# fjdf/slaMEM

Measured on AMD Instinct MI355X. Metric: MEMs/sec (and queries/sec) on 100 Mbp ref x 10 M 150 bp queries, l=20, higher is better.
Workload: dtype u32; 1 GPU; synthetic 100000000 bp reference (splitmix64 seed 42) x 10000000 reads/GPU of 150 bp, 2% substitutions, 50% reverse-complemented, -b -l 20; ref_len=100000000, reads_total=10000000, read_len=150, min_len=20, both_strands=True, parallelism=query shards x1, one GPU, no replication

## Files before the change

slamem_amd/csrc/mem_search.hip:

```cpp
#include "common.h"
#include "prims.h"

#include <atomic>
#include <type_traits>
#include <new>
#include <stdlib.h>
#include <string.h>

namespace slamem {

struct Blk {
    uint4 a;
    uint4 b;
    uint4 c;
    uint4 d;
};

__device__ __forceinline__ uint64_t u64_of(uint32_t lo, uint32_t hi) { return ((uint64_t)hi << 32) | lo; }

__device__ __forceinline__ Blk load_blk(const FMBlock* __restrict__ fm, uint32_t bi) {
    const uint4* p = reinterpret_cast<const uint4*>(fm + bi);
    Blk k;
    k.a = p[0]; k.b = p[1]; k.c = p[2]; k.d = p[3];
    return k;
// ... 102 lines not shown
struct SearchArgs {
    IndexView ix;
    const uint64_t* qwords;
    const uint64_t* offsets;
    uint32_t num_queries;
    uint32_t strands;
    uint32_t min_len;
    int32_t pad0;
    uint32_t pad1;
    uint32_t pad;
    uint64_t capacity;
    unsigned long long* total;
    RawKey* raw_key;
    slamem_mem* raw_mem;
    uint32_t* block_counts;
    struct RawRow* inline_rows;
    uint64_t inline_stride;
    const struct ItemDesc* items;
    uint64_t num_items;
    uint8_t* item_attempt;
    const uint8_t* item_alive;
    const uint32_t* work_ids;
    const uint32_t* work_count;
    unsigned long long* stats;
    uint64_t query_words;
    const uint64_t* pq;
    uint64_t* pq_out;
    uint32_t implicit_items;
    uint32_t* seed_left_ids;
    unsigned int* seed_left_count;
    unsigned int* seed_long_flag;
    unsigned int* seed_wide;
    uint32_t seed_step;
    const uint64_t* item_pk;
    unsigned int* work_cursor;
    int32_t direct_min_depth;
    uint32_t use_jump;
    uint32_t pad2;
    uint32_t skip_w;
    const uint64_t* pq2;
    uint64_t* pq2_out;
    uint8_t* item_flags;
    uint32_t skip_s1;
    uint32_t pad4;
    const struct SliceState* slice_state;
    const uint32_t* item_block;
    struct OutCtx {
        struct RawRow* inline_rows;
        uint64_t inline_stride;
        RawKey* raw_key;
        slamem_mem* raw_mem;
        unsigned long long* total;
        uint64_t capacity;
        uint32_t* block_counts;
        uint8_t* item_attempt;
    } prev;
    struct DeferCtx {
        struct JobRec* queue;
        unsigned int* njobs;
        uint32_t* pool;
        unsigned int* pool_next;
        uint32_t pool_cap;
        uint32_t queue_cap;
        uint32_t epoch;
        uint32_t* raw_seg;
        uint2* list;
        unsigned int* nlist;
        uint8_t* inline_valid;
    } defer;
    const struct CarryRec* carry_in;
    const unsigned int* carry_in_count;
    struct CarryRec* carry_out;
    unsigned int* carry_out_count;
};

struct RawRow { uint32_t row, pos, len; };
constexpr uint32_t kInlineMems = 4;
constexpr uint32_t kFetch = 64;

constexpr uint32_t kSliceLen = 4096;
static_assert(kSliceLen == kSearchSliceLen, "stream.hip tells the slice count of a batch from this length");
constexpr uint32_t kWarmUp = 1024;
constexpr uint32_t kMaxAttempt = 7;
struct __attribute__((aligned(16))) ItemDesc {
    uint64_t base;
    uint32_t len;
    uint32_t slice_rev;
};
__device__ __forceinline__ ItemDesc item_of(const SearchArgs& A, uint64_t it) {
    if (!A.implicit_items) return A.items[it];
    const uint64_t q = A.strands == 2u ? it >> 1 : it;
    const uint64_t o0 = A.offsets[q];
    return ItemDesc{o0, (uint32_t)(A.offsets[q + 1] - o0), A.strands == 2u ? (uint32_t)(it & 1ull) << 31 : 0u};
}
__device__ __forceinline__ uint64_t item_pk_of(const SearchArgs& A, uint64_t it, const ItemDesc& d) {
    if (!A.implicit_items) return A.item_pk[it];
    const uint64_t q = A.strands == 2u ? it >> 1 : it;
    const uint64_t rel = d.base - A.offsets[0];
    return 2ull + (uint64_t)A.strands * 2ull * ((rel >> 5) + q) + (uint64_t)(d.slice_rev >> 31) * 2ull * ((d.len + 31u) >> 5);
}

template <uint32_t kBytes>
struct QueryCursorT {
    const uint64_t* words;
    uint64_t base;
    uint32_t len;
    uint32_t rev;
    uint64_t cidx;
    uint64_t q0, q1, q2, q3;
    __device__ __forceinline__ void init(const uint64_t* q, uint64_t b, uint32_t l, uint32_t r) {
        words = q; base = b; len = l; rev = r; cidx = ~0ull;
// ... 2320 lines not shown
                    for (uint32_t wi = (af + s - 1u) / s, wl = (bf - k) / s; wi <= wl; wi++) {
                        const uint32_t x = st ? Lj - k - wi * s : wi * s;
                        uint64_t word = 0ull;
#pragma unroll
                        for (int w = 0; w < (int)NW; w++) word = (x >> 6) == (uint32_t)w ? uqs[w] : word;
                        if ((word >> (x & 63u)) & 1ull) done |= 1ull << wi;
                    }
                    if (done) atomicOr(&S.expl[jr], done);
                }
            }
            if (kStats) {
                const uint32_t nh = (uint32_t)__popcll(__ballot(has));
                n_cmp += nh;
                if (mark && lane == 0u) atomicAdd(A.stats + SC_SEED_ONCE, (unsigned long long)nh);
            }
            const unsigned long long mb = __ballot(is_mem);
            if (is_mem) {
                const uint32_t at = nmems + (uint32_t)__popcll(mb & below);
                if (at < SeedWave<NW, R>::kMems) { S.mem_key[at] = key; S.mem_ref[at] = ref; S.mem_sig[at] = sig | ((2u * jr + st) << 25); }
                else { atomicOr(&S.flags, 1u << jr); if (kStats) atomicAdd(A.stats + SC_SEED_WHY + 5u, 1ull); }
            }
            nmems += (uint32_t)__popcll(mb);
        }
        wave_sync();
    };

    for (uint32_t round = 0; round < (mstep > 1u ? 2u : 1u); round++) {
        njobs = 0;
        lookups(round);
        compares(round);
    }
    };
    if (wave_hasn) search(std::true_type{}); else search(std::false_type{});
    {
        if (nmems > SeedWave<NW, R>::kMems) nmems = SeedWave<NW, R>::kMems;

        const uint32_t g0 = (uint32_t)(r0 * strands);
        auto rank_of = [&](uint32_t mi, uint32_t key, uint32_t g, uint32_t& rank, uint32_t& cnt, bool& tie) {
            rank = 0; cnt = 0; tie = false;
            for (uint32_t t2 = 0; t2 < nmems; t2++) {
                const uint32_t kk = S.mem_key[t2], gg = S.mem_sig[t2] >> 25;
                const bool same = gg == g;
                cnt += same ? 1u : 0u;
                rank += (same && kk > key) ? 1u : 0u;
                tie = tie || (same && kk == key && t2 != mi);
            }
        };
        auto tie_rank = [&](uint32_t mi, uint32_t key, uint32_t myref, uint32_t g, uint32_t sig, uint32_t& rank) -> bool {
            const uint32_t a = key >> 16, b = a + (key & 0xFFFFu);
            bool child = false;
            for (uint32_t t2 = 0; t2 < nmems; t2++) {
                const uint32_t kk = S.mem_key[t2], a2 = kk >> 16, b2 = a2 + (kk & 0xFFFFu);
                child = child || ((S.mem_sig[t2] >> 25) == g && kk != key && a2 <= a && b2 > b);
            }
            const uint32_t jr = g >> 1, st = g & 1u;
            uint32_t qb = 0;
            if (child) qb = (uint32_t)((S.pl[jr][st][0][b >> 6] >> (b & 63u)) & 1ull) | ((uint32_t)((S.pl[jr][st][1][b >> 6] >> (b & 63u)) & 1ull) << 1);
            auto letter = [&](uint32_t sg, uint32_t t) { return ((sg >> t) & 1u) | (((sg >> (t + kSigLetters)) & 1u) << 1); };
            const bool rows = ix.prec != nullptr;
            const uint32_t my_side = child && letter(sig, 0u) > qb ? 1u : 0u;
            bool bad = (sig & kSigKnown) == 0u && (child || !rows);
            for (uint32_t t2 = 0; t2 < nmems; t2++) {
                const uint32_t so = S.mem_sig[t2];
                if (t2 == mi || (so >> 25) != g || S.mem_key[t2] != key) continue;
                const bool known = (so & sig & kSigKnown) != 0u;
                if (!known && (child || !rows)) { bad = true; continue; }
                const uint32_t o_side = child && letter(so, 0u) > qb ? 1u : 0u;
                bool before;
                if (o_side != my_side) before = o_side == 0u;
                else {
                    const uint32_t x = sig ^ so, diff = known ? (x | (x >> kSigLetters)) & kSigMask : 0u;
                    bool smaller;
                    if (diff != 0u) {
                        const uint32_t t = (uint32_t)__ffs((int)diff) - 1u;
                        smaller = letter(so, t) < letter(sig, t);
                    } else if (rows) smaller = ix.prec[S.mem_ref[t2]].row < ix.prec[myref].row;
                    else { bad = true; continue; }
                    before = my_side == 0u ? smaller : !smaller;
                }
                rank += before ? 1u : 0u;
            }
            return bad;
        };
        auto emit_mem = [&](uint32_t fl, uint32_t key, uint32_t ref, uint32_t gb, uint32_t rank, uint32_t cnt) {
            if ((fl >> (gb >> 1)) & 1u) return;
            const uint32_t g = g0 + (strands == 2u ? gb : gb >> 1);
            emit3_at(A, g, rank, 0u, ref, key >> 16, (key & 0xFFFFu) | 0x80000000u);
            if (rank == 0u) A.block_counts[g] = cnt;
            if (kStats) n_mem++;
        };
        if (nmems <= 64u) {
            const bool has = lane < nmems;
            const uint32_t key = has ? S.mem_key[lane] : 0u, ref = has ? S.mem_ref[lane] : 0u, g = has ? S.mem_sig[lane] >> 25 : 0xFFFFFFFFu;
            if (lane < 2u * R) S.smask[lane] = 0ull;
            wave_sync();
            if (has) atomicOr(&S.smask[g], 1ull << lane);
            wave_sync();
            const unsigned long long mine = has ? S.smask[g] : 0ull;
            uint32_t rank = 0;
            const uint32_t cnt = (uint32_t)__popcll(mine);
            bool tie = false;
            for (unsigned long long o = mine & ~(1ull << lane); __ballot(o != 0ull) != 0ull; o &= o - 1ull) {
                if (o == 0ull) continue;
                const uint32_t kk = S.mem_key[__ffsll(o) - 1];
                rank += kk > key ? 1u : 0u;
                tie = tie || kk == key;
            }
            if (has && tie && tie_rank(lane, key, ref, g, S.mem_sig[lane], rank)) {
                atomicOr(&S.flags, 1u << (g >> 1));
                if (kStats) atomicAdd(A.stats + SC_SEED_WHY + 6u, 1ull);
            }
            wave_sync();
            if (has) emit_mem(S.flags | wflags, key, ref, g, rank, cnt);
        } else {
            for (uint32_t pass = 0; pass < 2u; pass++) {
                const uint32_t fl = pass ? (S.flags | wflags) : 0u;
                for (uint32_t m0i = 0; m0i < nmems; m0i += 64u) {
                    const uint32_t mi = m0i + lane;
                    const bool has = mi < nmems;
                    const uint32_t key = has ? S.mem_key[mi] : 0u, ref = has ? S.mem_ref[mi] : 0u, g = has ? S.mem_sig[mi] >> 25 : 0xFFFFFFFFu;
                    uint32_t rank, cnt;
                    bool tie;
                    rank_of(mi, key, g, rank, cnt, tie);
                    const bool bad = has && tie && tie_rank(mi, key, ref, g, S.mem_sig[mi], rank);
                    if (!pass) { if (bad) atomicOr(&S.flags, 1u << (g >> 1)); }
                    else if (has) emit_mem(fl, key, ref, g, rank, cnt);
                }
                wave_sync();
            }
        }
    }
    wave_sync();
    const uint32_t fl = S.flags | wflags;
    {
        const bool isleft = lane < nr * strands && ((fl >> (strands == 2u ? lane >> 1 : lane)) & 1u) != 0u;
        if (lane < nr * strands) alive[r0 * strands + lane] = isleft ? 1 : 0;
        const unsigned long long lm = __ballot(isleft);
        if (lm != 0ull) {
            unsigned int at = 0;
            if (lane == 0u) at = atomicAdd(A.seed_left_count, (unsigned int)__popcll(lm));
            at = (unsigned int)__builtin_amdgcn_readfirstlane((int)at);
            if (isleft) A.seed_left_ids[at + (uint32_t)__popcll(lm & below)] = (uint32_t)(r0 * strands + lane);
        }
    }
    if (kStats) {
        stat_flush<kStats>(A.stats + SC_SEED_NMASKS, n_nm);
        stat_flush<kStats>(A.stats + SC_SEED_MEMS, n_mem);
        if (lane == 0u) {
            atomicAdd(A.stats + SC_SEED_WINDOWS, (unsigned long long)n_win);
            atomicAdd(A.stats + SC_SEED_COMPARES, (unsigned long long)n_cmp);
            atomicAdd(A.stats + SC_SEED_READS, (unsigned long long)nr);
            atomicAdd(A.stats + SC_SEED_QBYTES, (unsigned long long)(__builtin_amdgcn_readlane((int)(uint32_t)off, (int)nr) - __builtin_amdgcn_readlane((int)(uint32_t)off, 0)));
            atomicAdd(A.stats + SC_SEED_LEFT, (unsigned long long)(strands * (uint32_t)__popc(fl)));
            atomicAdd(A.stats + SC_SEED_WHY + 0u, (unsigned long long)__popc(wflags));
        }
    }
}

__global__ void __launch_bounds__(256) k_place_inline(const RawRow* __restrict__ inl, uint64_t stride, const uint32_t* __restrict__ counts,
                                                      const uint64_t* __restrict__ item_off, uint64_t nitems,
                                                      const uint32_t* __restrict__ sa, uint64_t capacity,
                                                      slamem_mem* __restrict__ out, const uint8_t* __restrict__ inline_valid) {
    uint64_t g = (uint64_t)blockIdx.x * blockDim.x + threadIdx.x;
    if (g >= nitems) return;
    uint32_t cnt = counts[g];
    uint64_t off = item_off[g];
    uint32_t iv = inline_valid ? inline_valid[g] : 0u;
    asm volatile("" : "+v"(cnt), "+v"(off), "+v"(iv));
    if (cnt > kInlineMems) cnt = kInlineMems;
    if (iv && cnt > iv - 1u) cnt = iv - 1u;
    if (cnt == 0u) return;
    static_assert(kInlineMems == 4, "k_place_inline is written for four inline slots");
    const RawRow* in = inl + g;
    const RawRow none = {0u, 0u, 0x80000000u};
    RawRow r0 = in[0], r1 = none, r2 = none, r3 = none;
    if (cnt > 1u) r1 = in[stride];
    if (cnt > 2u) r2 = in[2u * stride];
    if (cnt > 3u) r3 = in[3u * stride];
    asm volatile("" : "+v"(r0.row), "+v"(r0.pos), "+v"(r0.len), "+v"(r1.row), "+v"(r1.pos), "+v"(r1.len));
    asm volatile("" : "+v"(r2.row), "+v"(r2.pos), "+v"(r2.len), "+v"(r3.row), "+v"(r3.pos), "+v"(r3.len));
    uint32_t p0 = r0.row, p1 = r1.row, p2 = r2.row, p3 = r3.row;
    if (!(r0.len >> 31)) p0 = sa[r0.row];
    if (cnt > 1u && !(r1.len >> 31)) p1 = sa[r1.row];
    if (cnt > 2u && !(r2.len >> 31)) p2 = sa[r2.row];
    if (cnt > 3u && !(r3.len >> 31)) p3 = sa[r3.row];
    asm volatile("" : "+v"(p0), "+v"(p1), "+v"(p2), "+v"(p3));
    if (off < capacity) out[off] = slamem_mem{p0, r0.pos, r0.len & 0x7FFFFFFFu};
    if (cnt > 1u && off + 1u < capacity) out[off + 1u] = slamem_mem{p1, r1.pos, r1.len & 0x7FFFFFFFu};
    if (cnt > 2u && off + 2u < capacity) out[off + 2u] = slamem_mem{p2, r2.pos, r2.len & 0x7FFFFFFFu};
    if (cnt > 3u && off + 3u < capacity) out[off + 3u] = slamem_mem{p3, r3.pos, r3.len & 0x7FFFFFFFu};
}

__global__ void __launch_bounds__(256) k_group_totals(const uint32_t* __restrict__ counts, uint64_t nitems, uint64_t* __restrict__ totals) {
    const uint64_t g = (uint64_t)blockIdx.x * blockDim.x + threadIdx.x;
    uint64_t v = g < nitems ? (uint64_t)counts[g] : 0ull;
#pragma unroll
    for (int d = 32; d > 0; d >>= 1) v += u64_of(__shfl_down((uint32_t)v, d), __shfl_down((uint32_t)(v >> 32), d));
    if ((threadIdx.x & 63u) == 0u && (g >> 6) <= (nitems >> 6)) totals[g >> 6] = v;
}
__global__ void __launch_bounds__(256) k_place_grouped(const uint32_t* __restrict__ counts, uint64_t nitems, const uint64_t* __restrict__ group_prefix,
                                                       uint64_t* __restrict__ block_offsets, const RawRow* __restrict__ inl, uint64_t stride,
                                                       const uint32_t* __restrict__ sa, uint64_t capacity, slamem_mem* __restrict__ out,
                                                       const uint8_t* __restrict__ inline_valid) {
    const uint64_t g = (uint64_t)blockIdx.x * blockDim.x + threadIdx.x;
    const uint32_t lane = threadIdx.x & 63u;
    const bool item = g < nitems;
    const uint32_t full = item ? counts[g] : 0u;
    uint32_t iv = (item && inline_valid) ? inline_valid[g] : 0u;
    uint64_t gp = g <= nitems ? group_prefix[g >> 6] : 0ull;
    RawRow r0 = {0u, 0u, 0x80000000u};
    if (full != 0u) r0 = inl[g];
    asm volatile("" : "+v"(iv), "+v"(gp), "+v"(r0.row), "+v"(r0.pos), "+v"(r0.len));
    uint64_t incl = full;
#pragma unroll
    for (int d = 1; d < 64; d <<= 1) {
        const uint64_t o = u64_of(__shfl_up((uint32_t)incl, d), __shfl_up((uint32_t)(incl >> 32), d));
        if ((int)lane >= d) incl += o;
    }
    const uint64_t off = gp + (incl - full);
    if (g <= nitems) block_offsets[g] = off;
    uint32_t cnt = full > kInlineMems ? kInlineMems : full;
    if (iv && cnt > iv - 1u) cnt = iv - 1u;
    if (cnt == 0u) return;
    static_assert(kInlineMems == 4, "k_place_grouped is written for four inline slots");
    const RawRow none = {0u, 0u, 0x80000000u};
    RawRow r1 = none, r2 = none, r3 = none;
    if (cnt > 1u) r1 = inl[stride + g];
    if (cnt > 2u) r2 = inl[2u * stride + g];
    if (cnt > 3u) r3 = inl[3u * stride + g];
    asm volatile("" : "+v"(r1.row), "+v"(r1.pos), "+v"(r1.len), "+v"(r2.row), "+v"(r2.pos), "+v"(r2.len), "+v"(r3.row), "+v"(r3.pos), "+v"(r3.len));
    uint32_t p0 = r0.row, p1 = r1.row, p2 = r2.row, p3 = r3.row;
    if (!(r0.len >> 31)) p0 = sa[r0.row];
    if (cnt > 1u && !(r1.len >> 31)) p1 = sa[r1.row];
    if (cnt > 2u && !(r2.len >> 31)) p2 = sa[r2.row];
    if (cnt > 3u && !(r3.len >> 31)) p3 = sa[r3.row];
    asm volatile("" : "+v"(p0), "+v"(p1), "+v"(p2), "+v"(p3));
    if (off < capacity) out[off] = slamem_mem{p0, r0.pos, r0.len & 0x7FFFFFFFu};
    if (cnt > 1u && off + 1u < capacity) out[off + 1u] = slamem_mem{p1, r1.pos, r1.len & 0x7FFFFFFFu};
    if (cnt > 2u && off + 2u < capacity) out[off + 2u] = slamem_mem{p2, r2.pos, r2.len & 0x7FFFFFFFu};
    if (cnt > 3u && off + 3u < capacity) out[off + 3u] = slamem_mem{p3, r3.pos, r3.len & 0x7FFFFFFFu};
}

__global__ void __launch_bounds__(256) k_place_overflow(const RawKey* __restrict__ key, const slamem_mem* __restrict__ raw,
                                                        const unsigned long long* __restrict__ listed,
                                                        const uint64_t* __restrict__ item_off,
                                                        const uint8_t* __restrict__ item_attempt,
                                                        const uint32_t* __restrict__ sa, uint64_t capacity,
                                                        slamem_mem* __restrict__ out, const uint32_t* __restrict__ raw_seg,
                                                        const uint32_t* __restrict__ pool) {
    uint64_t count = *listed;
    if (count > capacity) count = capacity;
    const uint64_t stride = (uint64_t)gridDim.x * blockDim.x;
    for (uint64_t i = (uint64_t)blockIdx.x * blockDim.x + threadIdx.x; i < count; i += stride) {
        RawKey kk = key[i];
        if (kk.block == 0xFFFFFFFFu) continue;
        if ((kk.k >> 28) != item_attempt[kk.block]) continue;
        slamem_mem m = raw[i];
        uint64_t pos = item_off[kk.block] + (kk.k & 0x0FFFFFFFu);
        if (raw_seg) {
            const uint32_t sg = raw_seg[i];
            if (sg != 0xFFFFFFFFu) pos += pool[sg];
        }
        if (pos >= capacity) continue;
        if (m.length >> 31) m.length &= 0x7FFFFFFFu;
        else m.ref_pos = sa[m.ref_pos];
        out[pos] = m;
    }
}

__global__ void __launch_bounds__(256) k_item_counts(const uint64_t* __restrict__ offsets, uint32_t nq, uint32_t slice_len,
                                                     uint32_t* __restrict__ cnt, uint32_t* __restrict__ wps,
                                                     unsigned int* __restrict__ most) {
    uint64_t q = (uint64_t)blockIdx.x * blockDim.x + threadIdx.x;
    uint32_t c = 0, w = 0;
    if (q < nq) {
// ... 57 lines not shown
    uint32_t t = top[i], b = bot[i];
    if (t > b || b > ix.n) { depth_out[i] = -2; return; }
    depth_out[i] = parent(ix, t, b);
    top[i] = t;
    bot[i] = b;
}

__global__ void __launch_bounds__(256) k_locate_batch(IndexView ix, const uint32_t* __restrict__ rows, uint32_t* out,
                                                      uint64_t count) {
    uint64_t i = (uint64_t)blockIdx.x * blockDim.x + threadIdx.x;
    if (i >= count) return;
    uint32_t r = rows[i];
    out[i] = r <= ix.n ? ix.sa[r] : 0xFFFFFFFFu;
}

__global__ void __launch_bounds__(256) k_bwtchar_batch(IndexView ix, const uint32_t* __restrict__ rows, char* out,
                                                       uint64_t count) {
    uint64_t i = (uint64_t)blockIdx.x * blockDim.x + threadIdx.x;
    if (i >= count) return;
    uint32_t r = rows[i];
    const char L[] = {'$', 'N', 'A', 'C', 'G', 'T'};
    out[i] = r <= ix.n ? L[bwt_code(ix, r)] : '?';
}

namespace {
inline unsigned grid_for(uint64_t items, unsigned block = 256) { return (unsigned)((items + block - 1) / block); }
inline uint64_t align_up(uint64_t x, uint64_t a) { return (x + a - 1) / a * a; }

constexpr uint64_t kK8Waves = 4096;
constexpr uint64_t kCarryLanes = kK8Waves * 64;

struct WorkspaceLayout {
    uint64_t off_total, off_cnt, off_first, off_scan32, off_items, off_counts, off_attempt, off_alive, off_workids, off_select, select_bytes, off_itemoff, off_gsum, off_gpre, off_rawkey,
        off_rawmem, off_inline, off_scan, scan_bytes, off_wps, off_wscan, off_itempk, off_pq, pq_bytes, off_pq2, off_itemflags, off_mamstate, off_mamrun, off_itemblock, off_slicestate, off_carry, off_defscal, off_jobq, off_pool, off_rawseg, off_deflist, pool_cap, max_bounds, max_items, bytes;
};

WorkspaceLayout layout_workspace(uint64_t num_queries, uint64_t strands, uint64_t query_bytes, uint64_t capacity) {
    WorkspaceLayout w;
    w.max_items = strands * (num_queries + query_bytes / kSliceLen + 1);
    uint64_t off = 0;
    w.off_total = off;    off = align_up(off + 64 + SC_COUNT * 8, 256);
    w.off_cnt = off;      off = align_up(off + (num_queries + 2) * 4, 256);
    w.off_first = off;    off = align_up(off + (num_queries + 2) * 4, 256);
    w.off_scan32 = off;   off = align_up(off + scan_u32_tmp_words(num_queries + 1) * 4, 256);
    w.off_items = off;    off = align_up(off + w.max_items * sizeof(ItemDesc), 256);
    w.off_counts = off;   off = align_up(off + (w.max_items + 1) * 4, 256);
    w.off_attempt = off;  off = align_up(off + w.max_items, 256);
    w.off_alive = off;    off = align_up(off + w.max_items, 256);
    w.off_workids = off;  off = align_up(off + w.max_items * 4, 256);
    {
        size_t need2 = 0;
        (void)select_indices_u32(nullptr, need2, nullptr, nullptr, nullptr, w.max_items, 0);
        w.select_bytes = need2;
        w.off_select = off;
        off = align_up(off + need2, 256);
    }
    w.off_itemoff = off;  off = align_up(off + (w.max_items + 1) * 8, 256);
    w.off_gsum = off;     off = align_up(off + ((w.max_items >> 6) + 2) * 8, 256);
    w.off_gpre = off;     off = align_up(off + ((w.max_items >> 6) + 2) * 8, 256);
    w.off_rawkey = off;   off = align_up(off + capacity * sizeof(RawKey), 256);
    w.off_rawmem = off;   off = align_up(off + capacity * sizeof(slamem_mem), 256);
    w.off_inline = off;   off = align_up(off + w.max_items * kInlineMems * sizeof(RawRow), 256);
    size_t need = 0;
    (void)scan_sum_exclusive_u32_u64(nullptr, need, nullptr, nullptr, w.max_items, 0);
    w.scan_bytes = need;
    w.off_scan = off;     off = align_up(off + need, 256);
    w.off_wps = off;      off = align_up(off + (num_queries + 2) * 4, 256);
    w.off_wscan = off;    off = align_up(off + (num_queries + 2) * 8, 256);
    w.off_itempk = off;   off = align_up(off + w.max_items * 8, 256);
    w.pq_bytes = 8 * (4 + strands * (query_bytes / 16 + 2 * num_queries + 2));
    w.off_pq = off;       off = align_up(off + w.pq_bytes, 256);
    w.off_pq2 = off;      off = align_up(off + w.pq_bytes / 2 + 64, 256);
    w.off_itemflags = off; off = align_up(off + w.max_items, 256);
    w.max_bounds = strands * (query_bytes / kSliceLen + 1);
    w.off_mamstate = off; off = align_up(off + 2 * w.max_bounds * sizeof(MamState), 256);
    w.off_mamrun = off;   off = align_up(off + w.max_bounds * 4, 256);
    w.off_itemblock = off; off = align_up(off + w.max_items * 4, 256);
    w.off_slicestate = off; off = align_up(off + w.max_bounds * sizeof(SliceState), 256);
    w.off_carry = off;    off = align_up(off + kCarryLanes * sizeof(CarryRec), 256);
    w.pool_cap = strands * (query_bytes + 6 * num_queries) + 64;
    if (w.pool_cap > (32ull << 20)) w.pool_cap = 32ull << 20;
    w.off_defscal = off;  off = align_up(off + 64, 256);
    w.off_jobq = off;     off = align_up(off + (w.pool_cap + 64 * kK8Waves) * sizeof(JobRec), 256);
    w.off_pool = off;     off = align_up(off + (w.pool_cap + 16) * 4, 256);
    w.off_rawseg = off;   off = align_up(off + capacity * 4, 256);
    w.off_deflist = off;  off = align_up(off + w.max_items * 8, 256);
    w.bytes = off;
    return w;
}
}

uint64_t find_mems_workspace_bytes(uint64_t num_queries, int both_strands, uint64_t query_bytes, uint64_t mems_capacity) {
    return layout_workspace(num_queries, both_strands ? 2 : 1, query_bytes, mems_capacity).bytes;
}

static bool mam_whole_strands() {
    static const bool on = [] { const char* v = getenv("SLAMEM_MAM_WHOLE"); return v && atoi(v) != 0; }();
    return on;
}

struct SearchJob {
    const slamem_index* idx = nullptr;
    const void* queries_dev = nullptr;
    const uint64_t* offsets_dev = nullptr;
    uint32_t num_queries = 0, min_len = 0, strands = 1;
    uint64_t query_bytes = 0, mems_capacity = 0, workspace_bytes = 0, num_blocks = 0, nitems = 0, total = 0;
    int both_strands = 0, match_type = 0;
    slamem_mem* mems_dev = nullptr;
    uint64_t* block_offsets_dev = nullptr;
    void* workspace_dev = nullptr;
    WorkspaceLayout w;
    SearchArgs A;
    hipEvent_t ev[6] = {nullptr, nullptr, nullptr, nullptr, nullptr, nullptr};
    bool want_stats = false, prefiltered = false, timed_k8 = false, launched = false;
    bool rawkey_marked = false;
    bool deferred = false;
    bool speculate = false;
    bool speculated = false, saw_long = false;
    bool seed_path = false;
    bool seeded = false;
    uint32_t seed_words = 0, seed_words_avg = 0;
    bool mam_v3 = false;
    const FilterDesc* filter = nullptr;
    FilterParams params = {};
    FilterBatch batch = {};
    slamem_mem* out_mems = nullptr;
    uint64_t* out_boff = nullptr;
    void* filter_ws = nullptr;
    unsigned long long mum_large = 0;
    hipEvent_t ev_mum[2] = {nullptr, nullptr};
    uint64_t aln_totals[3] = {0, 0, 0};
    unsigned long long scal_own[16] = {0, 0, 0, 0, 0, 0, 0, 0, 0, 0, 0, 0, 0, 0, 0, 0};
    uint32_t k8_wave_cap = 0;
    uint32_t slices_hint = 0xFFFFFFFFu;
    unsigned long long* h_scal = scal_own;
    ~SearchJob();
    int init(const slamem_index* idx_, const void* queries_dev_, const uint64_t* offsets_dev_, uint32_t num_queries_,
             uint64_t query_bytes_, uint32_t min_len_, int both_strands_, int match_type_, slamem_mem* mems_dev_,
             uint64_t mems_capacity_, uint64_t* block_offsets_dev_, void* workspace_dev_, uint64_t workspace_bytes_,
             const FilterParams* params_);
    int tables(hipStream_t stream);
    int prep(hipStream_t stream);
    int search(hipStream_t stream) { int rc = search_k8(stream, nullptr, false); return rc != SLAMEM_OK ? rc : place(stream); }
    int search_k8(hipStream_t stream, SearchJob* carry_from, bool carry_out);
    bool enum_chunks() const;
    bool can_carry() const;
    bool can_carry_into(const SearchJob& next) const;
    int flush(hipStream_t stream);
    int place(hipStream_t stream);
    int collect();
    int finish(hipStream_t stream);
    bool carried_out = false;
    bool chunked = false;
// ... 189 lines not shown
            A.skip_w = 0;
            if (env_skip && kd && min_len >= kd && min_len >= 9u && min_len < 0x10000u && A.direct_min_depth >= 0) {
                const uint32_t s1 = min_len - kd + 1u;
                const uint32_t nprobes = (kd - 1u + s1 - 1u) / s1 + 1u;
                if (nprobes <= 4u && depth_class((int)min_len - 1) >= 1u) {
                    A.skip_w = min_len - 1u;
                    A.skip_s1 = s1;
                    A.pq2 = reinterpret_cast<const uint64_t*>(ws + w.off_pq2);
                    A.pq2_out = reinterpret_cast<uint64_t*>(ws + w.off_pq2);
                    A.item_flags = reinterpret_cast<uint8_t*>(ws + w.off_itemflags);
                }
            }
        }
    }
    return SLAMEM_OK;
}

int SearchJob::prep(hipStream_t stream) {
    SLAMEM_HIP(hipSetDevice(idx->device));
    char* ws = static_cast<char*>(workspace_dev);
    unsigned long long* d_total = reinterpret_cast<unsigned long long*>(ws + w.off_total);
    uint32_t* d_counts = reinterpret_cast<uint32_t*>(ws + w.off_counts);
    prefiltered = false; timed_k8 = false; launched = true; seeded = false; rawkey_marked = false;
    (void)hipEventRecord(ev[0], stream);
    if (nitems && (match_type != 1 || mam_v3)) {
        static const bool use_filter = [] { const char* v = getenv("SLAMEM_KFILTER"); return !(v && atoi(v) == 0); }();
        seeded = seed_path;
        if (seeded) {
            uint8_t* d_alive = reinterpret_cast<uint8_t*>(ws + w.off_alive);
            if (mems_capacity && !A.skip_w && !want_stats && enum_chunks()) {
                STEP(hipMemsetAsync(ws + w.off_rawkey, 0xFF, mems_capacity * sizeof(RawKey), stream), "memset");
                rawkey_marked = true;
            }
            STEP(hipMemsetAsync(d_counts, 0, nitems * 4, stream), "memset");
            STEP(hipMemsetAsync(A.item_attempt, 0, nitems, stream), "memset");
            {
                const char* v = getenv("SLAMEM_SEED_STEP");
                A.seed_step = v && atoi(v) >= 1 && atoi(v) <= 6 ? (uint32_t)atoi(v) : 0u;
            }
            uint32_t* d_ids = reinterpret_cast<uint32_t*>(ws + w.off_workids);
            uint32_t* d_nwork = reinterpret_cast<uint32_t*>(d_total) + 8;
            A.seed_left_ids = d_ids;
            A.seed_left_count = d_nwork;
            A.seed_long_flag = reinterpret_cast<unsigned int*>(d_total) + 3;
            A.seed_wide = reinterpret_cast<unsigned int*>(d_total) + 4;
            seed_words_avg = query_bytes > (uint64_t)num_queries * kSeedMaxLenMid ? 6u : query_bytes > (uint64_t)num_queries * kSeedMaxLen ? 4u : 3u;
            const uint32_t hint = __atomic_load_n(&idx->seed_words_hint, __ATOMIC_RELAXED);
            seed_words = seed_words_avg > hint ? seed_words_avg : hint;
            const bool mid_reads = seed_words == 4u, long_reads = seed_words == 6u;
            const dim3 gs(grid_for((uint64_t)num_queries, 4 * (long_reads ? kSeedReadsLong : mid_reads ? kSeedReadsMid : kSeedReads)));
            if (long_reads) {
                if (want_stats) hipLaunchKernelGGL((k_seed_mems<true, 6, kSeedReadsLong>), gs, dim3(256), 0, stream, A, d_alive);
                else hipLaunchKernelGGL((k_seed_mems<false, 6, kSeedReadsLong>), gs, dim3(256), 0, stream, A, d_alive);
            } else if (mid_reads) {
                if (want_stats) hipLaunchKernelGGL((k_seed_mems<true, 4, kSeedReadsMid>), gs, dim3(256), 0, stream, A, d_alive);
                else hipLaunchKernelGGL((k_seed_mems<false, 4, kSeedReadsMid>), gs, dim3(256), 0, stream, A, d_alive);
            } else {
                if (want_stats) hipLaunchKernelGGL((k_seed_mems<true, 3, kSeedReads>), gs, dim3(256), 0, stream, A, d_alive);
                else hipLaunchKernelGGL((k_seed_mems<false, 3, kSeedReads>), gs, dim3(256), 0, stream, A, d_alive);
            }
            STEP(hipGetLastError(), "k_seed_mems");
            (void)hipEventRecord(ev[3], stream);
            prefiltered = true;
            A.item_alive = d_alive;
            A.work_ids = d_ids;
            A.work_count = d_nwork;
            if (use_filter && idx->view.kfilter && min_len >= idx->view.kfilter_k) {
                hipLaunchKernelGGL(k_prefilter_list, dim3(512), dim3(256), 0, stream, A, (const uint32_t*)d_ids, (const uint32_t*)d_nwork, d_alive);
                STEP(hipGetLastError(), "k_prefilter_list");
            }
        } else if (use_filter && idx->view.kfilter && min_len >= idx->view.kfilter_k) {
            uint8_t* d_alive = reinterpret_cast<uint8_t*>(ws + w.off_alive);
            if (want_stats) hipLaunchKernelGGL(k_prefilter<true>, dim3(grid_for(nitems)), dim3(256), 0, stream, A, d_alive);
            else hipLaunchKernelGGL(k_prefilter<false>, dim3(grid_for(nitems)), dim3(256), 0, stream, A, d_alive);
            STEP(hipGetLastError(), "k_prefilter");
            (void)hipEventRecord(ev[3], stream);
            prefiltered = true;
            A.item_alive = d_alive;
            STEP(hipMemsetAsync(d_counts, 0, nitems * 4, stream), "memset");
            STEP(hipMemsetAsync(A.item_attempt, 0, nitems, stream), "memset");
            uint32_t* d_ids = reinterpret_cast<uint32_t*>(ws + w.off_workids);
            uint32_t* d_nwork = reinterpret_cast<uint32_t*>(d_total) + 8;
            size_t need2 = w.select_bytes;
// ... 214 lines not shown
                STEP(hipMemsetAsync(d_nrun, 0, 4, stream), "memset");
                hipLaunchKernelGGL(k_mam_check, dim3(grid_for(nitems)), dim3(256), 0, stream, A, P, d_run, d_nrun);
                STEP(hipGetLastError(), "k_mam_check");
                STEP(hipMemcpyAsync(&nrun, d_nrun, 4, hipMemcpyDeviceToHost, stream), "memcpy");
                STEP(hipStreamSynchronize(stream), "k_mam_check (sync)");
                if (nrun == 0) break;
                reruns += nrun; passes++;
                MamPass R = P;
                R.run_list = d_run;
                R.run_count = d_nrun;
                hipLaunchKernelGGL(k_find_mams_sliced, dim3(grid_for(nrun)), dim3(256), 0, stream, A, R);
                STEP(hipGetLastError(), "k_find_mams_sliced (rerun)");
            }
            if (env_trace)
                fprintf(stderr, "[mam] %llu slices of %llu strands, warm-up %u: %llu scanned again in %llu passes\n", (unsigned long long)nitems,
                        (unsigned long long)num_blocks, env_warm, (unsigned long long)reruns, (unsigned long long)passes);
        }
    }
    (void)hipEventRecord(ev[1], stream);
    return SLAMEM_OK;
}

int SearchJob::place(hipStream_t stream) {
    SLAMEM_HIP(hipSetDevice(idx->device));
    if (carried_out) { set_error("internal: K9 before the batch's last lanes are finished"); return SLAMEM_ERR_ARG; }
    char* ws = static_cast<char*>(workspace_dev);
    unsigned long long* d_total = reinterpret_cast<unsigned long long*>(ws + w.off_total);
    uint32_t* d_first = reinterpret_cast<uint32_t*>(ws + w.off_first);
    uint32_t* d_counts = reinterpret_cast<uint32_t*>(ws + w.off_counts);
    const bool blocks_are_items = nitems == num_blocks;
    uint64_t* d_itemoff = blocks_are_items ? block_offsets_dev : reinterpret_cast<uint64_t*>(ws + w.off_itemoff);
    size_t need = w.scan_bytes;
    const bool grouped = blocks_are_items && nitems && mems_capacity && [] { const char* v = getenv("SLAMEM_K9_GROUPED"); return !(v && atoi(v) == 0); }();
    if (grouped) {
        const uint64_t ngroups = (nitems >> 6) + 1;
        uint64_t* d_gsum = reinterpret_cast<uint64_t*>(ws + w.off_gsum);
        uint64_t* d_gpre = reinterpret_cast<uint64_t*>(ws + w.off_gpre);
        STEP(hipMemsetAsync(d_gsum + ngroups, 0, 8, stream), "memset");
        hipLaunchKernelGGL(k_group_totals, dim3(grid_for(ngroups * 64)), dim3(256), 0, stream, (const uint32_t*)d_counts, nitems, d_gsum);
        STEP(hipGetLastError(), "k_group_totals");
        STEP(scan_sum_exclusive_u64(ws + w.off_scan, need, d_gsum, d_gpre, ngroups, stream), "scan");
        hipLaunchKernelGGL(k_place_grouped, dim3(grid_for(nitems + 1)), dim3(256), 0, stream, (const uint32_t*)d_counts, nitems, (const uint64_t*)d_gpre,
                           block_offsets_dev, (const RawRow*)A.inline_rows, A.inline_stride, idx->view.sa, mems_capacity, mems_dev,
                           deferred ? (const uint8_t*)A.defer.inline_valid : (const uint8_t*)nullptr);
        STEP(hipGetLastError(), "k_place_grouped");
    } else {
        STEP(scan_sum_exclusive_u32_u64(ws + w.off_scan, need, d_counts, d_itemoff, nitems, stream), "scan");
    }
    if (!blocks_are_items) {
        hipLaunchKernelGGL(k_block_offsets, dim3(grid_for(num_blocks + 1)), dim3(256), 0, stream, d_first, d_itemoff,
                           num_queries, strands, nitems, block_offsets_dev);
        STEP(hipGetLastError(), "k_block_offsets");
    }
    if (nitems && mems_capacity) {
        if (!grouped) {
            hipLaunchKernelGGL(k_place_inline, dim3(grid_for(nitems)), dim3(256), 0, stream, A.inline_rows, A.inline_stride, d_counts,
                               d_itemoff, nitems, idx->view.sa, mems_capacity, mems_dev, deferred ? (const uint8_t*)A.defer.inline_valid : (const uint8_t*)nullptr);
            STEP(hipGetLastError(), "k_place_inline");
        }
        const uint64_t ob = (mems_capacity + 255) / 256;
        hipLaunchKernelGGL(k_place_overflow, dim3((unsigned)(ob < 2048 ? ob : 2048)), dim3(256), 0, stream, A.raw_key, A.raw_mem,
                           (const unsigned long long*)d_total, d_itemoff, A.item_attempt, idx->view.sa, mems_capacity, mems_dev,
                           deferred ? (const uint32_t*)A.defer.raw_seg : (const uint32_t*)nullptr, deferred ? (const uint32_t*)A.defer.pool : (const uint32_t*)nullptr);
        STEP(hipGetLastError(), "k_place_overflow");
    }
    (void)hipEventRecord(ev[2], stream);
    STEP(hipMemcpyAsync(h_scal, d_total, 8 * sizeof(unsigned long long), hipMemcpyDeviceToHost, stream), "memcpy");
    STEP(hipMemcpyAsync(h_scal + 8, d_itemoff + nitems, 8, hipMemcpyDeviceToHost, stream), "memcpy");
    if (filter) {
        (void)hipEventRecord(ev_mum[0], stream);
        int rc = filter->run(filter_ws, batch, params, out_mems, out_boff, h_scal + 9, stream);
        if (rc != SLAMEM_OK) return rc;
// ... 223 lines not shown
```

Measured before the change: 5.082 billion MEMs/s.

## Stage seed MEMs in per-wave contiguous runs and place them with a grouped kernel

The seed kernel now gathers each wave's MEMs into a contiguous per-wave staging slot, ordered by strand with a wave prefix sum. It no longer scatters them through the strided inline rows, and it writes block counts, attempt bytes and a per-strand mark itself. A new placement kernel scans the counts per seed group and copies each run straight to the output with coalesced stores, falling back to inline rows for strands that overflowed. This removes two memsets and the strided inline traffic and SA lookups. In exchange it adds a staging buffer and more complex owner-mapping logic in placement.

```diff
diff --git a/slamem_amd/csrc/mem_search.hip b/slamem_amd/csrc/mem_search.hip
--- a/slamem_amd/csrc/mem_search.hip
+++ b/slamem_amd/csrc/mem_search.hip
@@ -158,6 +158,7 @@
     unsigned int* seed_long_flag;
     unsigned int* seed_wide;
     uint32_t seed_step;
+    struct RawRow* run_rows;
     const uint64_t* item_pk;
     unsigned int* work_cursor;
     int32_t direct_min_depth;
@@ -203,6 +204,9 @@
 struct RawRow { uint32_t row, pos, len; };
 constexpr uint32_t kInlineMems = 4;
 constexpr uint32_t kFetch = 64;
+constexpr uint32_t kRunRows = 128;
+static_assert((kRunRows * sizeof(RawRow)) % 64u == 0u, "a slot of the staging area is a whole number of 64-byte lines");
+constexpr uint8_t kStrandInRun = 0, kStrandLeft = 1, kStrandInline = 2;
 
 constexpr uint32_t kSliceLen = 4096;
 static_assert(kSliceLen == kSearchSliceLen, "stream.hip tells the slice count of a batch from this length");
@@ -2589,6 +2593,7 @@
     }
     };
     if (wave_hasn) search(std::true_type{}); else search(std::false_type{});
+    uint32_t run_cnt = 0, run_at = 0, run_fit = 1u, nrun = 0;
     {
         if (nmems > SeedWave<NW, R>::kMems) nmems = SeedWave<NW, R>::kMems;
 
@@ -2639,11 +2644,26 @@
             }
             return bad;
         };
-        auto emit_mem = [&](uint32_t fl, uint32_t key, uint32_t ref, uint32_t gb, uint32_t rank, uint32_t cnt) {
-            if ((fl >> (gb >> 1)) & 1u) return;
-            const uint32_t g = g0 + (strands == 2u ? gb : gb >> 1);
-            emit3_at(A, g, rank, 0u, ref, key >> 16, (key & 0xFFFFu) | 0x80000000u);
-            if (rank == 0u) A.block_counts[g] = cnt;
+        static_assert(SeedWave<NW, R>::kJobs >= kRunRows && 2u * R <= 64u, "the run is put together in the compares' lists, a lane per strand");
+        auto settle = [&](uint32_t c) {
+            run_cnt = c;
+            uint32_t incl = c;
+#pragma unroll
+            for (int d = 1; d < 64; d <<= 1) {
+                const uint32_t o = __shfl_up(incl, d);
+                if ((int)lane >= d) incl += o;
+            }
+            run_at = incl - c;
+            run_fit = (A.run_rows != nullptr && incl <= kRunRows) ? 1u : 0u;
+            const unsigned long long fm = __ballot(run_fit != 0u);
+            nrun = fm != 0ull ? (uint32_t)__shfl(incl, (int)__popcll(fm) - 1) : 0u;
+        };
+        auto put_mem = [&](bool on, uint32_t fl, uint32_t key, uint32_t ref, uint32_t gb, uint32_t rank) {
+            const uint32_t at = (uint32_t)__shfl(run_at, (int)(on ? gb : 0u)) + rank;
+            const bool fit = __shfl(run_fit, (int)(on ? gb : 0u)) != 0u;
+            if (!on || ((fl >> (gb >> 1)) & 1u) != 0u) return;
+            if (fit) { S.job_p[at] = ref; S.job_x[at] = key; }
+            else emit3_at(A, g0 + (strands == 2u ? gb : gb >> 1), rank, 0u, ref, key >> 16, (key & 0xFFFFu) | 0x80000000u);
             if (kStats) n_mem++;
         };
         if (nmems <= 64u) {
@@ -2655,7 +2675,6 @@
             wave_sync();
             const unsigned long long mine = has ? S.smask[g] : 0ull;
             uint32_t rank = 0;
-            const uint32_t cnt = (uint32_t)__popcll(mine);
             bool tie = false;
             for (unsigned long long o = mine & ~(1ull << lane); __ballot(o != 0ull) != 0ull; o &= o - 1ull) {
                 if (o == 0ull) continue;
@@ -2668,10 +2687,18 @@
                 if (kStats) atomicAdd(A.stats + SC_SEED_WHY + 6u, 1ull);
             }
             wave_sync();
-            if (has) emit_mem(S.flags | wflags, key, ref, g, rank, cnt);
+            const uint32_t fl = S.flags | wflags;
+            settle(lane < 2u * R && ((fl >> (lane >> 1)) & 1u) == 0u ? (uint32_t)__popcll(S.smask[lane]) : 0u);
+            put_mem(has, fl, key, ref, g, rank);
         } else {
             for (uint32_t pass = 0; pass < 2u; pass++) {
                 const uint32_t fl = pass ? (S.flags | wflags) : 0u;
+                if (pass) {
+                    uint32_t c = 0;
+                    if (lane < 2u * R && ((fl >> (lane >> 1)) & 1u) == 0u)
+                        for (uint32_t t2 = 0; t2 < nmems; t2++) c += (S.mem_sig[t2] >> 25) == lane ? 1u : 0u;
+                    settle(c);
+                }
                 for (uint32_t m0i = 0; m0i < nmems; m0i += 64u) {
                     const uint32_t mi = m0i + lane;
                     const bool has = mi < nmems;
@@ -2681,7 +2708,7 @@
                     rank_of(mi, key, g, rank, cnt, tie);
                     const bool bad = has && tie && tie_rank(mi, key, ref, g, S.mem_sig[mi], rank);
                     if (!pass) { if (bad) atomicOr(&S.flags, 1u << (g >> 1)); }
-                    else if (has) emit_mem(fl, key, ref, g, rank, cnt);
+                    else put_mem(has, fl, key, ref, g, rank);
                 }
                 wave_sync();
             }
@@ -2690,8 +2717,22 @@
     wave_sync();
     const uint32_t fl = S.flags | wflags;
     {
+        RawRow* slot = A.run_rows + (uint64_t)(blockIdx.x * 4u + wv) * kRunRows;
+        for (uint32_t i = lane; i < nrun; i += 64u) {
+            const uint32_t key = S.job_x[i];
+            slot[i] = RawRow{S.job_p[i], key >> 16, key & 0xFFFFu};
+        }
+    }
+    {
+        const uint32_t sb = (strands == 2u ? lane : 2u * lane) & 63u;
+        const uint32_t scnt = (uint32_t)__shfl(run_cnt, (int)sb), sfit = (uint32_t)__shfl(run_fit, (int)sb);
         const bool isleft = lane < nr * strands && ((fl >> (strands == 2u ? lane >> 1 : lane)) & 1u) != 0u;
-        if (lane < nr * strands) alive[r0 * strands + lane] = isleft ? 1 : 0;
+        if (lane < nr * strands) {
+            const uint64_t g = r0 * strands + lane;
+            alive[g] = isleft ? kStrandLeft : (scnt != 0u && sfit == 0u) ? kStrandInline : kStrandInRun;
+            A.block_counts[g] = scnt;
+            A.item_attempt[g] = 0;
+        }
         const unsigned long long lm = __ballot(isleft);
         if (lm != 0ull) {
             unsigned int at = 0;
@@ -2748,12 +2789,16 @@
     if (cnt > 3u && off + 3u < capacity) out[off + 3u] = slamem_mem{p3, r3.pos, r3.len & 0x7FFFFFFFu};
 }
 
-__global__ void __launch_bounds__(256) k_group_totals(const uint32_t* __restrict__ counts, uint64_t nitems, uint64_t* __restrict__ totals) {
-    const uint64_t g = (uint64_t)blockIdx.x * blockDim.x + threadIdx.x;
-    uint64_t v = g < nitems ? (uint64_t)counts[g] : 0ull;
+__global__ void __launch_bounds__(256) k_group_totals(const uint32_t* __restrict__ counts, uint64_t nitems, uint32_t per, uint64_t ngroups,
+                                                      uint64_t* __restrict__ totals) {
+    const uint64_t grp = (uint64_t)blockIdx.x * 4u + (threadIdx.x >> 6);
+    const uint32_t lane = threadIdx.x & 63u;
+    if (grp >= ngroups) return;
+    const uint64_t g = grp * per + lane;
+    uint64_t v = (lane < per && g < nitems) ? (uint64_t)counts[g] : 0ull;
 #pragma unroll
     for (int d = 32; d > 0; d >>= 1) v += u64_of(__shfl_down((uint32_t)v, d), __shfl_down((uint32_t)(v >> 32), d));
-    if ((threadIdx.x & 63u) == 0u && (g >> 6) <= (nitems >> 6)) totals[g >> 6] = v;
+    if (lane == 0u) totals[grp] = v;
 }
 __global__ void __launch_bounds__(256) k_place_grouped(const uint32_t* __restrict__ counts, uint64_t nitems, const uint64_t* __restrict__ group_prefix,
                                                        uint64_t* __restrict__ block_offsets, const RawRow* __restrict__ inl, uint64_t stride,
@@ -2798,6 +2843,78 @@
     if (cnt > 3u && off + 3u < capacity) out[off + 3u] = slamem_mem{p3, r3.pos, r3.len & 0x7FFFFFFFu};
 }
 
+__global__ void __launch_bounds__(256) k_place_runs(const uint32_t* __restrict__ counts, const uint8_t* __restrict__ marks, uint64_t nitems,
+                                                    uint32_t per, uint64_t ngroups, const uint64_t* __restrict__ group_prefix,
+                                                    uint64_t* __restrict__ block_offsets, const RawRow* __restrict__ runs,
+                                                    const RawRow* __restrict__ inl, uint64_t stride, const uint32_t* __restrict__ sa,
+                                                    uint64_t capacity, slamem_mem* __restrict__ out, const uint8_t* __restrict__ inline_valid) {
+    const uint64_t grp = (uint64_t)blockIdx.x * 4u + (threadIdx.x >> 6);
+    const uint32_t lane = threadIdx.x & 63u;
+    if (grp >= ngroups) return;
+    const uint64_t g = grp * per + lane;
+    const bool item = lane < per && g < nitems;
+    const uint32_t full = item ? counts[g] : 0u;
+    const uint32_t mark = item ? (uint32_t)marks[g] : 0u;
+    uint32_t iv = (item && inline_valid) ? inline_valid[g] : 0u;
+    const uint64_t gp = group_prefix[grp];
+    const RawRow* src = runs + grp * kRunRows;
+    RawRow first = src[lane];
+    asm volatile("" : "+v"(iv), "+v"(first.row), "+v"(first.pos), "+v"(first.len));
+    const uint32_t inrun = mark == kStrandInRun ? full : 0u;
+    uint64_t incl = full;
+    uint32_t incl_in = inrun;
+#pragma unroll
+    for (int d = 1; d < 64; d <<= 1) {
+        const uint64_t o = u64_of(__shfl_up((uint32_t)incl, d), __shfl_up((uint32_t)(incl >> 32), d));
+        const uint32_t oi = __shfl_up(incl_in, d);
+        if ((int)lane >= d) { incl += o; incl_in += oi; }
+    }
+    const uint64_t off = gp + (incl - full);
+    if (item) block_offsets[g] = off;
+    if (grp + 1u == ngroups && lane == 63u) block_offsets[nitems] = gp + incl;
+    uint32_t nrun = (uint32_t)__shfl(incl_in, 63);
+    if (nrun > kRunRows) nrun = kRunRows;
+    if (__ballot(mark != kStrandInRun && full != 0u) == 0ull) {
+        for (uint32_t i = lane; i < nrun; i += 64u) {
+            const RawRow r = i < 64u ? first : src[i];
+            if (gp + i < capacity) out[gp + i] = slamem_mem{r.row, r.pos, r.len};
+        }
+        return;
+    }
+    for (uint32_t ib = 0; ib < nrun; ib += 64u) {
+        const uint32_t i = ib + lane;
+        uint32_t owner = 0;
+        for (uint32_t t = 0; t < per; t++) owner += (uint32_t)__shfl(incl_in, (int)t) <= i ? 1u : 0u;
+        owner = owner < per ? owner : per - 1u;
+        const uint64_t o_off = u64_of(__shfl((uint32_t)off, (int)owner), __shfl((uint32_t)(off >> 32), (int)owner));
+        const uint32_t o_at = (uint32_t)__shfl(incl_in - inrun, (int)owner);
+        const uint64_t pos = o_off + (i - o_at);
+        if (i >= nrun) continue;
+        const RawRow r = i < 64u ? first : src[i];
+        if (pos < capacity) out[pos] = slamem_mem{r.row, r.pos, r.len};
+    }
+    uint32_t cnt = mark != kStrandInRun ? (full > kInlineMems ? kInlineMems : full) : 0u;
+    if (iv && cnt > iv - 1u) cnt = iv - 1u;
+    if (cnt == 0u) return;
+    static_assert(kInlineMems == 4, "k_place_runs is written for four inline slots");
+    const RawRow none = {0u, 0u, 0x80000000u};
+    RawRow r0 = inl[g], r1 = none, r2 = none, r3 = none;
+    if (cnt > 1u) r1 = inl[stride + g];
+    if (cnt > 2u) r2 = inl[2u * stride + g];
+    if (cnt > 3u) r3 = inl[3u * stride + g];
+    asm volatile("" : "+v"(r0.row), "+v"(r0.pos), "+v"(r0.len), "+v"(r1.row), "+v"(r1.pos), "+v"(r1.len));
+    asm volatile("" : "+v"(r2.row), "+v"(r2.pos), "+v"(r2.len), "+v"(r3.row), "+v"(r3.pos), "+v"(r3.len));
+    uint32_t p0 = r0.row, p1 = r1.row, p2 = r2.row, p3 = r3.row;
+    if (!(r0.len >> 31)) p0 = sa[r0.row];
+    if (cnt > 1u && !(r1.len >> 31)) p1 = sa[r1.row];
+    if (cnt > 2u && !(r2.len >> 31)) p2 = sa[r2.row];
+    if (cnt > 3u && !(r3.len >> 31)) p3 = sa[r3.row];
+    if (off < capacity) out[off] = slamem_mem{p0, r0.pos, r0.len & 0x7FFFFFFFu};
+    if (cnt > 1u && off + 1u < capacity) out[off + 1u] = slamem_mem{p1, r1.pos, r1.len & 0x7FFFFFFFu};
+    if (cnt > 2u && off + 2u < capacity) out[off + 2u] = slamem_mem{p2, r2.pos, r2.len & 0x7FFFFFFFu};
+    if (cnt > 3u && off + 3u < capacity) out[off + 3u] = slamem_mem{p3, r3.pos, r3.len & 0x7FFFFFFFu};
+}
+
 __global__ void __launch_bounds__(256) k_place_overflow(const RawKey* __restrict__ key, const slamem_mem* __restrict__ raw,
                                                         const unsigned long long* __restrict__ listed,
                                                         const uint64_t* __restrict__ item_off,
@@ -2921,7 +3038,7 @@
 
 struct WorkspaceLayout {
     uint64_t off_total, off_cnt, off_first, off_scan32, off_items, off_counts, off_attempt, off_alive, off_workids, off_select, select_bytes, off_itemoff, off_gsum, off_gpre, off_rawkey,
-        off_rawmem, off_inline, off_scan, scan_bytes, off_wps, off_wscan, off_itempk, off_pq, pq_bytes, off_pq2, off_itemflags, off_mamstate, off_mamrun, off_itemblock, off_slicestate, off_carry, off_defscal, off_jobq, off_pool, off_rawseg, off_deflist, pool_cap, max_bounds, max_items, bytes;
+        off_rawmem, off_inline, off_runs, off_scan, scan_bytes, off_wps, off_wscan, off_itempk, off_pq, pq_bytes, off_pq2, off_itemflags, off_mamstate, off_mamrun, off_itemblock, off_slicestate, off_carry, off_defscal, off_jobq, off_pool, off_rawseg, off_deflist, pool_cap, max_bounds, max_items, bytes;
 };
 
 WorkspaceLayout layout_workspace(uint64_t num_queries, uint64_t strands, uint64_t query_bytes, uint64_t capacity) {
@@ -2945,11 +3062,12 @@
         off = align_up(off + need2, 256);
     }
     w.off_itemoff = off;  off = align_up(off + (w.max_items + 1) * 8, 256);
-    w.off_gsum = off;     off = align_up(off + ((w.max_items >> 6) + 2) * 8, 256);
-    w.off_gpre = off;     off = align_up(off + ((w.max_items >> 6) + 2) * 8, 256);
+    w.off_gsum = off;     off = align_up(off + ((w.max_items >> 4) + 3) * 8, 256);
+    w.off_gpre = off;     off = align_up(off + ((w.max_items >> 4) + 3) * 8, 256);
     w.off_rawkey = off;   off = align_up(off + capacity * sizeof(RawKey), 256);
     w.off_rawmem = off;   off = align_up(off + capacity * sizeof(slamem_mem), 256);
     w.off_inline = off;   off = align_up(off + w.max_items * kInlineMems * sizeof(RawRow), 256);
+    w.off_runs = off;     off = align_up(off + (num_queries / (kSeedReads < kSeedReadsMid ? kSeedReads : kSeedReadsMid) + 1) * kRunRows * sizeof(RawRow), 256);
     size_t need = 0;
     (void)scan_sum_exclusive_u32_u64(nullptr, need, nullptr, nullptr, w.max_items, 0);
     w.scan_bytes = need;
@@ -3008,6 +3126,8 @@
     bool speculated = false, saw_long = false;
     bool seed_path = false;
     bool seeded = false;
+    bool use_runs = false;
+    uint32_t seed_reads = 0;
     uint32_t seed_words = 0, seed_words_avg = 0;
     bool mam_v3 = false;
     const FilterDesc* filter = nullptr;
@@ -3263,8 +3383,8 @@
                 STEP(hipMemsetAsync(ws + w.off_rawkey, 0xFF, mems_capacity * sizeof(RawKey), stream), "memset");
                 rawkey_marked = true;
             }
-            STEP(hipMemsetAsync(d_counts, 0, nitems * 4, stream), "memset");
-            STEP(hipMemsetAsync(A.item_attempt, 0, nitems, stream), "memset");
+            use_runs = mems_capacity != 0 && [] { const char* v = getenv("SLAMEM_K9_GROUPED"); return !(v && atoi(v) == 0); }();
+            A.run_rows = use_runs ? reinterpret_cast<RawRow*>(ws + w.off_runs) : nullptr;
             {
                 const char* v = getenv("SLAMEM_SEED_STEP");
                 A.seed_step = v && atoi(v) >= 1 && atoi(v) <= 6 ? (uint32_t)atoi(v) : 0u;
@@ -3279,7 +3399,8 @@
             const uint32_t hint = __atomic_load_n(&idx->seed_words_hint, __ATOMIC_RELAXED);
             seed_words = seed_words_avg > hint ? seed_words_avg : hint;
             const bool mid_reads = seed_words == 4u, long_reads = seed_words == 6u;
-            const dim3 gs(grid_for((uint64_t)num_queries, 4 * (long_reads ? kSeedReadsLong : mid_reads ? kSeedReadsMid : kSeedReads)));
+            seed_reads = long_reads ? kSeedReadsLong : mid_reads ? kSeedReadsMid : kSeedReads;
+            const dim3 gs(grid_for((uint64_t)num_queries, 4 * seed_reads));
             if (long_reads) {
                 if (want_stats) hipLaunchKernelGGL((k_seed_mems<true, 6, kSeedReadsLong>), gs, dim3(256), 0, stream, A, d_alive);
                 else hipLaunchKernelGGL((k_seed_mems<false, 6, kSeedReadsLong>), gs, dim3(256), 0, stream, A, d_alive);
@@ -3560,12 +3681,26 @@
     uint64_t* d_itemoff = blocks_are_items ? block_offsets_dev : reinterpret_cast<uint64_t*>(ws + w.off_itemoff);
     size_t need = w.scan_bytes;
     const bool grouped = blocks_are_items && nitems && mems_capacity && [] { const char* v = getenv("SLAMEM_K9_GROUPED"); return !(v && atoi(v) == 0); }();
-    if (grouped) {
+    if (grouped && seeded && use_runs) {
+        const uint32_t per = seed_reads * strands;
+        const uint64_t ngroups = (nitems + per - 1) / per;
+        uint64_t* d_gsum = reinterpret_cast<uint64_t*>(ws + w.off_gsum);
+        uint64_t* d_gpre = reinterpret_cast<uint64_t*>(ws + w.off_gpre);
+        STEP(hipMemsetAsync(d_gsum + ngroups, 0, 8, stream), "memset");
+        hipLaunchKernelGGL(k_group_totals, dim3(grid_for(ngroups * 64)), dim3(256), 0, stream, (const uint32_t*)d_counts, nitems, per, ngroups, d_gsum);
+        STEP(hipGetLastError(), "k_group_totals");
+        STEP(scan_sum_exclusive_u64(ws + w.off_scan, need, d_gsum, d_gpre, ngroups, stream), "scan");
+        hipLaunchKernelGGL(k_place_runs, dim3(grid_for(ngroups * 64)), dim3(256), 0, stream, (const uint32_t*)d_counts,
+                           (const uint8_t*)(ws + w.off_alive), nitems, per, ngroups, (const uint64_t*)d_gpre, block_offsets_dev,
+                           (const RawRow*)A.run_rows, (const RawRow*)A.inline_rows, A.inline_stride, idx->view.sa, mems_capacity, mems_dev,
+                           deferred ? (const uint8_t*)A.defer.inline_valid : (const uint8_t*)nullptr);
+        STEP(hipGetLastError(), "k_place_runs");
+    } else if (grouped) {
         const uint64_t ngroups = (nitems >> 6) + 1;
         uint64_t* d_gsum = reinterpret_cast<uint64_t*>(ws + w.off_gsum);
         uint64_t* d_gpre = reinterpret_cast<uint64_t*>(ws + w.off_gpre);
         STEP(hipMemsetAsync(d_gsum + ngroups, 0, 8, stream), "memset");
-        hipLaunchKernelGGL(k_group_totals, dim3(grid_for(ngroups * 64)), dim3(256), 0, stream, (const uint32_t*)d_counts, nitems, d_gsum);
+        hipLaunchKernelGGL(k_group_totals, dim3(grid_for(ngroups * 64)), dim3(256), 0, stream, (const uint32_t*)d_counts, nitems, 64u, ngroups, d_gsum);
         STEP(hipGetLastError(), "k_group_totals");
         STEP(scan_sum_exclusive_u64(ws + w.off_scan, need, d_gsum, d_gpre, ngroups, stream), "scan");
         hipLaunchKernelGGL(k_place_grouped, dim3(grid_for(nitems + 1)), dim3(256), 0, stream, (const uint32_t*)d_counts, nitems, (const uint64_t*)d_gpre,
```

Result: slower. 4.984 billion MEMs/s (-1.9%).
